# aukeschaap/ttcross

Measured on AMD Instinct MI355X. Metric: fiber evals/s (neval / wall time of dtt_dmrgg), Ising C_64 n=51 r=32 piv=2 (d=63), higher is better.
Workload: dtype f64; 1 GPU; Ising C_64 n=51 r=32 piv=2 (d=63); driver=test_crs_ising c 64 51 32 2, bond_groups=8, transport=none (single process), arith=exact, sweeps=16

## Files before the change

### ttcross_amd/csrc/ttx_cluster.h

```cpp
#pragma once
#include "ttx_fused.h"
#include "ttx_mvn.h"

#define CB 256
#ifndef TTX_CL_UNR
#define TTX_CL_UNR 16
#endif

__device__ __forceinline__ double f_ising_c4p(int m, int A, const double *an, const double *aw, double s1n, double s1w,
                                              double s2n, double s2w, const double *bn, const double *bw,
                                              double pv, double pvk, double pw, double pwk)
{
    const int nb = m - A - 2;
    double v = pv, w = pw, vk = pvk, wk = pwk;
    auto vstep = [&](double xv) { vk = vk * xv; v = v + vk; };
    auto wstep = [&](double xv) { wk = wk * xv; w = w + wk; };
    vstep(s2n); vstep(s1n);
    chain8v<true>(an, A, vstep);
    wstep(s1n); wstep(s2n);
    chain8v<false>(bn, nb, wstep);
    double b = 1.0 / (v * w);
    double f = 2 * b;
    auto fstep = [&](double xv) { f = f * xv; };
    chain8v<false>(aw, A, fstep);
    fstep(s1w); fstep(s2w);
    chain8v<false>(bw, nb, fstep);
    return f;
}

template <class STEP>
__device__ __forceinline__ void chain8w(const double *p, int nc, STEP step)
{
#pragma unroll 1
    for (int ch = 0; ch < nc; ch++) {
        double x[8];
        ld8d(p + 8 * ch, x);
#pragma unroll
        for (int k = 0; k < 8; k++) step(x[k]);
    }
}
__device__ __forceinline__ double f_ising_c4w(int cA, int cB, const double *an, const double *aw, double s1n, double s1w,
                                              double s2n, double s2w, const double *bn, const double *bw,
                                              double pv, double pvk, double pw, double pwk)
{
    double v = pv, w = pw, vk = pvk, wk = pwk;
    auto vstep = [&](double xv) { vk = vk * xv; v = v + vk; };
    auto wstep = [&](double xv) { wk = wk * xv; w = w + wk; };
    vstep(s2n); vstep(s1n);
    chain8w(an, cA, vstep);
    wstep(s1n); wstep(s2n);
    chain8w(bn, cB, wstep);
    double b = 1.0 / (v * w);
    double f = 2 * b;
    auto fstep = [&](double xv) { f = f * xv; };
    chain8w(aw, cA, fstep);
    fstep(s1w); fstep(s2w);
    chain8w(bw, cB, fstep);
    return f;
}

__device__ __forceinline__ int wave_min_i(int v)
{
    v = min(v, __builtin_amdgcn_update_dpp(INT_MAX, v, 0xb1, 0xf, 0xf, false));
    v = min(v, __builtin_amdgcn_update_dpp(INT_MAX, v, 0x4e, 0xf, 0xf, false));
    v = min(v, __builtin_amdgcn_update_dpp(INT_MAX, v, 0x124, 0xf, 0xf, false));
    v = min(v, __builtin_amdgcn_update_dpp(INT_MAX, v, 0x128, 0xf, 0xf, false));
    v = min(v, __builtin_amdgcn_update_dpp(INT_MAX, v, 0x142, 0xa, 0xf, false));
    v = min(v, __builtin_amdgcn_update_dpp(INT_MAX, v, 0x143, 0xc, 0xf, false));
    return __builtin_amdgcn_readlane(v, 63);
}
__device__ __forceinline__ void wave_argmax2(double &a, double &v, int &idx)
{
    const double amx = wave_max(a);
    const int key = (a == amx && idx != INT_MAX) ? ((idx << 1) | (signbit(v) ? 1 : 0)) : INT_MAX;
    const int kmin = wave_min_i(key);
    a = amx;
    if (kmin == INT_MAX) { idx = INT_MAX; v = 0.0; }
    else { idx = kmin >> 1; v = (kmin & 1) ? -amx : amx; }
}

__device__ __forceinline__ double f_ising_cfast(double xj, double wj, double xk, double wk, double pv, double pvk, double pw, double pwk,
                                                double SL, double WL, double SR, double WR)
{
    const double v = pv + pvk * xk * (1.0 + xj * (1.0 + SL));
    const double w = pw + pwk * xj * (1.0 + xk * (1.0 + SR));
    return 2.0 / (v * w) * ((WL * wj) * (wk * WR));
}

typedef unsigned int u4 __attribute__((ext_vector_type(4)));
struct ClRec { u4 a, b; };
static_assert(sizeof(ClRec) == sizeof(ClPart), "record buffers are sized as ClPart: [2][G][TTX_CLREC] u4 arg-max records, then as many running-maximum records");
__device__ __forceinline__ void st16(void *p, u4 v) { asm volatile("global_store_dwordx4 %0, %1, off sc1" :: "v"(p), "v"(v) : "memory"); }
__device__ __forceinline__ u4 ld16(const void *p)
{
    u4 v;
    asm volatile("global_load_dwordx4 %0, %1, off sc1\n\ts_waitcnt vmcnt(0)" : "=v"(v) : "v"(p) : "memory");
    return v;
}

__device__ __forceinline__ int xcc_id() { return (int)__builtin_amdgcn_s_getreg(((4 - 1) << 11) | 20) & 15; }
__global__ void k_xcc_probe(int *out) { if (threadIdx.x == 0) out[blockIdx.x] = xcc_id(); }

__device__ __forceinline__ bool cluster_sync(unsigned *ctr, unsigned target, int *abortflag, int *s_ok)
{
    asm volatile("s_waitcnt vmcnt(0)" ::: "memory");
    __syncthreads();
    if (threadIdx.x == 0) {
        int ok = 1;
        unsigned spins = 0;
        __hip_atomic_fetch_add(ctr, 1u, __ATOMIC_RELEASE, __HIP_MEMORY_SCOPE_AGENT);
        while (__hip_atomic_load(ctr, __ATOMIC_RELAXED, __HIP_MEMORY_SCOPE_AGENT) < target) {
            __builtin_amdgcn_s_sleep(1);
            if (++spins > (1u << 22)) { ok = 0; __hip_atomic_store(abortflag, 1, __ATOMIC_RELAXED, __HIP_MEMORY_SCOPE_SYSTEM); break; }
            if ((spins & 1023u) == 0 && __hip_atomic_load(abortflag, __ATOMIC_RELAXED, __HIP_MEMORY_SCOPE_SYSTEM)) { ok = 0; break; }
        }
        __atomic_thread_fence(__ATOMIC_ACQUIRE);
        *s_ok = ok;
    }
    __syncthreads();
    return *s_ok != 0;
}

#ifdef TTX_STAMPS
#define CST_DECL const bool t_me = (threadIdx.x == 0 && g == 0 && cb == 0); long long t_prev = wall_clock64()
#define CST(k) do { if (t_me) { long long t_now = wall_clock64(); gs.stamp[0][k] += t_now - t_prev; t_prev = t_now; } } while (0)
#define CST_END() do { if (t_me) gs.nstamp[0]++; } while (0)
#define WST(k) do { if (P.dbg && g == 0 && epoch == 8 && pp == 4 && lane == 0 && h < 8) P.dbg[((size_t)(h * 64 + cb * 4 + wv)) * 8 + (k)] = (long long)__builtin_readcyclecounter(); } while (0)
#else
#define WST(k)
#define CST_DECL
#define CST(k)
#define CST_END()
#endif

template <bool CFAST, bool CPAD>
__global__ __launch_bounds__(CB) void k_sweep_cluster(DevProb P, int dir, int nsteps, int NB, int ldsinv, int epoch, int zkeep)
{
    extern __shared__ __align__(16) double dyn[];
    __shared__ int zc[128], zr[128], zcs[128], zrs[128], keepc[128], keepr[128];
    __shared__ int nzc, nzr, nsc, nsr, s_ok;
    __shared__ ttx_cdfseg segc[TTX_TABSEG], segr[TTX_TABSEG];
    __shared__ double sha[8], shv[8], shm[8]; __shared__ int shi[8];
    __shared__ double pLw[64], pLk[64], pRv[64], pRk[64];
    static_assert(!(CFAST && CPAD), "the closed form reads the rows in dimension order");
    constexpr int NFT = CFAST ? 64 : 1;
    __shared__ double fSL[NFT], fWL[NFT], fSR[NFT], fWR[NFT];
    __shared__ struct { int ii, jj, kk, qq, hcount, rc_k, rc_q, rr_i, rr_j; double pivot, amax, bytes_half; long long neval, n_resid; } s_rook;
    const int bid = blockIdx.x;
    const int g = (bid & 7) + 8 * (bid / (8 * NB)), cb = (bid >> 3) % NB;
    if (g >= P.G || P.ctl[0]) return;
    const int bpar = (epoch - 1) & 1;
    if (P.tail_side && epoch >= 2) {
        const TailRec &t0 = P.tailrec[(size_t)bpar * P.G];
        if (stop_rule(epoch - 1, P.maxrank, P.accuracy, t0.pivotmax, max_pos(t0.amax, P.gs[0].amax_bnd[bpar]), P.strk[epoch & 1]).ready) return;
    }
    if (P.cl_test_abort && P.cl_test_abort == epoch && g == 0 && cb == 0) {
        if (threadIdx.x == 0) { __hip_atomic_store(P.cl_abort, 1, __ATOMIC_RELAXED, __HIP_MEMORY_SCOPE_SYSTEM); P.ctl[0] = 1; }
        return;
    }
    const int tid = threadIdx.x, m = P.d, RM = P.RM, NM = P.NM;
    const int lane = tid & 63, wv = tid >> 6;
    GroupState &gs = P.gs[g];
    const int first = gs.first, last = gs.last, nbonds = last - first + 1;
    int *r = P.r + (size_t)g * (m + 2);
    const int VS = ((m + 7) & ~7) + 8;
    const int RS = 2 * VS + 2;
    const int n1m = P.n[1];
    const int SL = RM * ((NM + NB - 1) / NB + 1);
    unsigned *ctr = P.cl_ctr + g;
    unsigned nbar = (unsigned)(epoch - 1) * (unsigned)min(nsteps, nbonds);
    ClPart *part = P.cl_part;
    double *par = dyn;
    double *XL = par + ((P.npar + 1) & ~1);
    double *XR = XL + (size_t)RM * RS;
    double *acol = XR + (size_t)RM * RS;
    double *arow = acol + SL;
    double *resc = arow + SL;
    double *resr = resc + SL;
    double *xsc = resr + SL;
    double *xsr = xsc + ((RM + 1) & ~1);
    int *lot = (int *)(xsr + ((RM + 1) & ~1));
    double *GL = (double *)(lot + 4 * ((2 * RM + 2 * NM + 4 + 1) & ~1));
    double *GU = GL + (size_t)RM * RM;
    int *ZK = (int *)(ldsinv ? GU + (size_t)RM * RM : GL);
    int *ZN = ZK + (size_t)nsteps * 2 * RM;
    for (int x = tid; x < P.npar; x += CB) par[x] = P.par[x];
    if (cb == 0 && tid == 0) sweep_start(P, g);
    __syncthreads();
    if (zkeep) {
        int *TMP = (int *)XL;
        const int E = nbonds * 2 * RM;
        for (int x = tid; x < E; x += CB) {
            const int b = x / (2 * RM), side = (x / RM) & 1, u = x % RM, pb = first + b;
            if (u < r[pb]) { const int *vp = vip_ptr(P, g, pb, first) + 4 * u; TMP[x] = (vp[2 * side + 1] << 16) | vp[2 * side]; }
        }
        __syncthreads();
        for (int x = tid; x < E; x += CB) {
            const int b = x / (2 * RM), u = x % RM, nb_ = r[first + b];
            if (u < nb_) {
                const int *src = TMP + (x - u); const int a = src[u]; int ra = 0;
                for (int t = 0; t < nb_; t++) ra += (src[t] < a) || (src[t] == a && t < u);
                ZK[(x - u) + ra] = a;
            }
        }
        __syncthreads();
        for (int x = tid; x < E; x += CB) {
            const int b = x / (2 * RM), u = x % RM, nb_ = r[first + b];
            if (u < nb_) {
                const int *src = ZK + (x - u); int pc = 0;
                for (int t = 1; t <= u; t++) pc += (src[t] != src[t - 1]);
                const bool keep = (u == 0) || (src[u] != src[u - 1]);
                TMP[x] = keep ? pc : -1;
                if (u == nb_ - 1) ZN[x / RM] = pc + 1;
            }
        }
        __syncthreads();
        int mykey = 0, mypos = -1;
        for (int x0 = 0; x0 < E; x0 += CB) {
            const int x = x0 + tid;
            mypos = -1;
            if (x < E) { const int b = x / (2 * RM), u = x % RM; if (u < r[first + b]) { mypos = TMP[x]; mykey = ZK[x]; } }
            __syncthreads();
            if (mypos >= 0) ZK[(x - x % RM) + mypos] = mykey;
            __syncthreads();
        }
    }
    double amax = gs.amax, pivotmax = -1.0, pivotmin = -1.0;
    if (P.tail_side && epoch >= 2) amax = max_pos(amax, gs.amax_bnd[bpar]);
    const double pivotmax_prev = gs.pivotmax_prev;
    long long neval = gs.neval;
    unsigned long long rngpos = gs.rngpos;
    double bytes_half = gs.bytes_half; long long n_resid = gs.n_resid;
    int hcount = 0;
    const unsigned long long bil0 = ttx_minstd_pow(2ull * tid);
    unsigned long long sA0 = ttx_minstd_pow(2 * rngpos + 1);
    const int bl0 = (int)ttx_minstd_pow(2ull * lane);
    const unsigned long long c64 = ttx_minstd_pow(128);
    CST_DECL;

    for (int pp = 1; pp <= nsteps; pp++) {
        if (pp > nbonds) break;
        const int p = (dir == 1) ? first + pp - 1 : last + 1 - pp;
        const int r0 = r[p - 1], r1 = r[p], r2 = r[p + 1], n1 = P.n[p], n2 = P.n[p + 1];
        const int nlot = r0 + n1 + n2 + r2;
        auto slice = [&](int c, int n) { return (int)((unsigned)c * (unsigned)n / (unsigned)NB); };
        const int jlo = slice(cb, n1), jhi = slice(cb + 1, n1);
        const int klo = slice(cb, n2), khi = slice(cb + 1, n2);
        const int nj = jhi - jlo, nk = khi - klo;
        double *Cp = core_ptr(P, P.col, g, p, first), *Wq = core_ptr(P, P.row, g, p + 1, first);
        double *Ap = core_ptr(P, P.arg, g, p, first), *Aq = core_ptr(P, P.arg, g, p + 1, first);
        const short *Lt = L_ptr(P, g, p - 1, first), *Rt = R_ptr(P, g, p + 1, first);
        const int cA = (p - 1 + 7) >> 3, cB = (m - p - 1 + 7) >> 3;
        const int sside = (tid >> 6) & 1, sseg = tid & 63;
        double sg_a0 = 0.0, sg_al = 0.0, sg_de = 0.0; int sg_k0 = 0, sg_cn = 0, myns = 0;
        auto seg_issue = [&](int Kc_, int Kr_) {
            if (tid >= 128) {
                const int K = sside ? Kr_ : Kc_; const ttx_cdfseg *sp = P.cdf_tab + (size_t)K * TTX_TABSEG + sseg;
                myns = P.cdf_ns[K]; sg_a0 = sp->a0; sg_al = sp->alast; sg_de = sp->delta; sg_k0 = sp->k0; sg_cn = sp->cnt;
            }
        };
        {
            const int AL = min(VS, (p - 1 + 7) & ~7), AR = min(VS, (m - p - 1 + 7) & ~7);
            if (AL > 0) {
                int c = tid / AL, o = tid - c * AL;
                const int dc = CB / AL, dO = CB - dc * AL;
                while (c < r0) {
                    if constexpr (CPAD) {
                        if (o < p - 1) {
                            const int ix = (int)Lt[(size_t)o * RM + c];
                            XL[(size_t)c * RS + (p - 2 - o)] = par[ix - 1]; XL[(size_t)c * RS + VS + o] = par[n1m + ix - 1];
                        } else { XL[(size_t)c * RS + o] = 0.0; XL[(size_t)c * RS + VS + o] = 1.0; }
                    } else {
                        const int ix = (o < p - 1) ? (int)Lt[(size_t)o * RM + c] : 1;
                        XL[(size_t)c * RS + o] = par[ix - 1]; XL[(size_t)c * RS + VS + o] = par[n1m + ix - 1];
                    }
                    c += dc; o += dO; if (o >= AL) { o -= AL; c++; }
                }
            }
            if (AR > 0) {
                int c = tid / AR, o = tid - c * AR;
                const int dc = CB / AR, dO = CB - dc * AR;
                while (c < r2) {
                    if (CPAD && o >= m - p - 1) { XR[(size_t)c * RS + o] = 0.0; XR[(size_t)c * RS + VS + o] = 1.0; }
                    else {
                        const int ix = (o < m - p - 1) ? (int)Rt[(size_t)o * RM + c] : 1;
                        XR[(size_t)c * RS + o] = par[ix - 1]; XR[(size_t)c * RS + VS + o] = par[n1m + ix - 1];
                    }
                    c += dc; o += dO; if (o >= AR) { o -= AR; c++; }
                }
            }
        }
        if (ldsinv) {
            if (p > first) { const double *gL = inv_ptr(P, g, p - 1, first); for (int x = tid; x < r0 * r0; x += CB) GL[x] = gL[x]; }
            if (p < last)  { const double *gU = inv_ptr(P, g, p + 1, first); for (int x = tid; x < r2 * r2; x += CB) GU[x] = gU[x]; }
        }
        CST(0);
        if (zkeep) seg_issue(r0 * n1 - ZN[2 * (p - first)], n2 * r2 - ZN[2 * (p - first) + 1]);
        if (tid == 0) s_ok = 1;
        unsigned long long stepmul;
        if (nlot < 512) {
            stepmul = (unsigned long long)(unsigned)__shfl(bl0, nlot & 63);
            for (int a = 0; a < (nlot >> 6); a++) stepmul = ttx_mulmod31(stepmul, c64);
        } else stepmul = ttx_minstd_pow(2ull * nlot);
        const unsigned long long sA1 = ttx_mulmod31(sA0, stepmul);
        if (zkeep) {
            const int b = p - first;
            const int *kc = ZK + (size_t)b * 2 * RM, *kr = kc + RM;
            if (tid == 0) { nzc = ZN[2 * b]; nzr = ZN[2 * b + 1]; }
            if (tid < ZN[2 * b]) zc[tid] = ((kc[tid] & 0xffff) - 1) + r0 * ((kc[tid] >> 16) - 1) + 1;
            if (tid < ZN[2 * b + 1]) zr[tid] = ((kr[tid] & 0xffff) - 1) + n2 * ((kr[tid] >> 16) - 1) + 1;
            __syncthreads();
        } else bond_zero_lists(vip_ptr(P, g, p, first), r1, r0, n2, tid, zc, zr, zcs, zrs, keepc, keepr, &nzc, &nzr);
        CST(1);
        const int Kc = r0 * n1 - nzc, Kr = n2 * r2 - nzr;
        if (!zkeep) seg_issue(Kc, Kr);
        if (tid >= 128) {
            ttx_cdfseg *dst = sside ? segr : segc;
            if (sseg < myns) { dst[sseg].a0 = sg_a0; dst[sseg].alast = sg_al; dst[sseg].delta = sg_de; dst[sseg].k0 = sg_k0; dst[sseg].cnt = sg_cn; }
            if (sseg == 0) { if (sside) nsr = myns; else nsc = myns; }
        }
        if (tid < r0) {
            double w = 1.0, wk = 1.0;
            auto wstep = [&](double xv) { wk = wk * xv; w = w + wk; };
            if constexpr (CPAD) chain8v<true>(XL + (size_t)tid * RS, p - 1, wstep);
            else chain8v<false>(XL + (size_t)tid * RS, p - 1, wstep);
            pLw[tid] = w; pLk[tid] = wk;
            if constexpr (CFAST) {
                double sk = 1.0, ss = 0.0, ww = 1.0;
                auto sstep = [&](double xv) { sk = sk * xv; ss = ss + sk; };
                auto pstep = [&](double xv) { ww = ww * xv; };
                chain8v<true>(XL + (size_t)tid * RS, p - 1, sstep);
                chain8v<false>(XL + (size_t)tid * RS + VS, p - 1, pstep);
                fSL[tid] = ss; fWL[tid] = ww;
            }
        } else if (tid >= 64 && tid < 64 + r2) {
            const int c = tid - 64;
            double v = 1.0, vk = 1.0;
            auto vstep = [&](double xv) { vk = vk * xv; v = v + vk; };
            chain8v<true>(XR + (size_t)c * RS, m - p - 1, vstep);
            pRv[c] = v; pRk[c] = vk;
            if constexpr (CFAST) {
                double sk = 1.0, ss = 0.0, ww = 1.0;
                auto sstep = [&](double xv) { sk = sk * xv; ss = ss + sk; };
                auto pstep = [&](double xv) { ww = ww * xv; };
                chain8v<false>(XR + (size_t)c * RS, m - p - 1, sstep);
                chain8v<false>(XR + (size_t)c * RS + VS, m - p - 1, pstep);
                fSR[c] = ss; fWR[c] = ww;
            }
        }
        __syncthreads();
        CST(2);
        double ma = 0.0, ba = -1.0, bv = 0.0; int bi = INT_MAX;
        const int nscu = __builtin_amdgcn_readfirstlane(nsc), nsru = __builtin_amdgcn_readfirstlane(nsr);
        const int nzcu = __builtin_amdgcn_readfirstlane(nzc), nzru = __builtin_amdgcn_readfirstlane(nzr);
        for (int il = tid; il < nlot; il += CB) {
            const unsigned long long bil = (il == tid) ? bil0 : ttx_minstd_pow(2ull * il);
            const double d1 = ttx_flang_from_word(ttx_mulmod31(sA0, bil)), d2 = ttx_flang_from_word(ttx_mulmod31(sA1, bil));
            const ttx_pair xy = ttx_lottery_index2<TTX_TABSEG, 64>(segc, nscu, Kc, r0 * n1, zc, nzcu, d1, segr, nsru, Kr, n2 * r2, zr, nzru, d2);
            const int x = xy.x, y = xy.y;
            CST(3);
            const int i = (x - 1) % r0 + 1, j = (x - 1) / r0 + 1, k = (y - 1) % n2 + 1, q = (y - 1) / n2 + 1;
            lot[4 * il] = i; lot[4 * il + 1] = j; lot[4 * il + 2] = k; lot[4 * il + 3] = q;
            const double *rl = XL + (size_t)(i - 1) * RS, *rq = XR + (size_t)(q - 1) * RS;
            double f;
            if constexpr (CFAST) f = f_ising_cfast(par[j - 1], par[n1m + j - 1], par[k - 1], par[n1m + k - 1], pRv[q - 1], pRk[q - 1], pLw[i - 1], pLk[i - 1], fSL[i - 1], fWL[i - 1], fSR[q - 1], fWR[q - 1]);
            else if constexpr (CPAD) f = f_ising_c4w(cA, cB, rl, rl + VS, par[j - 1], par[n1m + j - 1], par[k - 1], par[n1m + k - 1], rq, rq + VS, pRv[q - 1], pRk[q - 1], pLw[i - 1], pLk[i - 1]);
            else f = f_ising_c4p(m, p - 1, rl, rl + VS, par[j - 1], par[n1m + j - 1], par[k - 1], par[n1m + k - 1], rq, rq + VS, pRv[q - 1], pRk[q - 1], pLw[i - 1], pLk[i - 1]);
            ma = fmax(ma, fabs(f));
            CST(4);
            const double *c = Cp + (i - 1) + (size_t)RM * (j - 1), *w = Wq + (k - 1) + (size_t)NM * (q - 1);
            double t = 0.0;
#pragma unroll 8
            for (int s = 0; s < r1; s++) t = t + c[P.SS * s] * w[P.SW * s];
            const double b = f - t, aa = fabs(b);
            if (aa > ba || (aa == ba && il < bi)) { ba = aa; bv = b; bi = il; }
        }
        ma = wave_max(ma);
        wave_argmax(ba, bv, bi);
        if (lane == 0) { shm[wv] = ma; sha[wv] = ba; shv[wv] = bv; shi[wv] = bi; }
        __syncthreads();
        ma = shm[0]; ba = sha[0]; bv = shv[0]; bi = shi[0];
        for (int x = 1; x < CB / 64; x++) {
            ma = fmax(ma, shm[x]);
            if (sha[x] > ba || (sha[x] == ba && shi[x] < bi)) { ba = sha[x]; bv = shv[x]; bi = shi[x]; }
        }
        amax = fmax(amax, ma);
        neval += nlot; rngpos += 2ull * nlot;
        sA0 = ttx_mulmod31(sA1, stepmul);
        if (bi == INT_MAX) bi = 0;
        int ii = lot[4 * bi], jj = lot[4 * bi + 1], kk = lot[4 * bi + 2], qq = lot[4 * bi + 3];
        double pivot = bv;
        CST(5);
        int havecol = 0, haverow = 0, crs = 0, done = 0;
        int rc_k = -1, rc_q = -1, rr_i = -1, rr_j = -1;
        const int H = (P.piv == 0) ? 2 : 2 * P.piv;
        const int r1u = __builtin_amdgcn_readfirstlane(r1);
        double mxrun = 0.0;
        auto wact = [&](int c) {
            const int njc = slice(c + 1, n1) - slice(c, n1), nkc = slice(c + 1, n2) - slice(c, n2);
            const int e = max(r0 * njc, nkc * r2);
            return min(CB / 64, max(1, (e + 63) >> 6));
        };
        const bool rook_active = wv < wact(cb);
        const bool slot_on = (lane < NB * (CB / 64)) && ((lane & (CB / 64 - 1)) < wact(lane / (CB / 64)));
        if (rook_active) {
        for (int h = 0; h < H && !done; h++) {
            const bool iscol = (P.piv == 0) ? (h == 0) : (((h + (dir == 2 ? 1 : 0)) & 1) == 0);
            const int nf = iscol ? r0 * n1 : n2 * r2;
            const int nsl = iscol ? r0 * nj : nk * r2;
            double *fib = iscol ? acol : arow;
            double xsv = 0.0;
            if (lane < r1) xsv = iscol ? Wq[(kk - 1) + (size_t)NM * (qq - 1) + P.SW * lane] : Cp[(ii - 1) + (size_t)RM * (jj - 1) + P.SS * lane];
            crs++;
            if (iscol) havecol = 1; else haverow = 1;
            const int dn = (P.piv == 0) ? (h == 1) : (havecol && haverow && (crs >= 2 * P.piv));
            const bool resid = (P.piv != 0) && !dn;
            if (iscol) { rc_k = resid ? kk : -1; rc_q = qq; } else { rr_i = resid ? ii : -1; rr_j = jj; }
            CST(6);
            WST(0);
            double mx = 0.0, ab = -1.0, bb = 0.0; int ix = INT_MAX;
            for (int u = tid; u < nsl; u += CB) {
                double a;
                if (iscol) {
                    const int i = u % r0, j = jlo + u / r0, t = i + r0 * j;
                    const double *rl = XL + (size_t)i * RS, *rq = XR + (size_t)(qq - 1) * RS;
                    const double *c = Cp + i + (size_t)RM * j;
                    if constexpr (CFAST) a = f_ising_cfast(par[j], par[n1m + j], par[kk - 1], par[n1m + kk - 1], pRv[qq - 1], pRk[qq - 1], pLw[i], pLk[i], fSL[i], fWL[i], fSR[qq - 1], fWR[qq - 1]);
                    else if constexpr (CPAD) a = f_ising_c4w(cA, cB, rl, rl + VS, par[j], par[n1m + j], par[kk - 1], par[n1m + kk - 1], rq, rq + VS, pRv[qq - 1], pRk[qq - 1], pLw[i], pLk[i]);
                    else a = f_ising_c4p(m, p - 1, rl, rl + VS, par[j], par[n1m + j], par[kk - 1], par[n1m + kk - 1], rq, rq + VS, pRv[qq - 1], pRk[qq - 1], pLw[i], pLk[i]);
                    fib[u] = a;
                    if (resid) {
                        double b = a;
#pragma unroll TTX_CL_UNR
                        for (int s = 0; s < r1u; s++) b = b + (-mvn_lane(xsv, s)) * c[P.SS * s];
                        resc[u] = b;
                        const double aa = fabs(b);
                        if (aa > ab || (aa == ab && t < ix)) { ab = aa; bb = b; ix = t; }
                    }
                } else {
                    const int k = klo + u % nk, q = u / nk, t = k + n2 * q;
                    const double *rl = XL + (size_t)(ii - 1) * RS, *rq = XR + (size_t)q * RS;
                    const double *w = Wq + k + (size_t)NM * q;
                    if constexpr (CFAST) a = f_ising_cfast(par[jj - 1], par[n1m + jj - 1], par[k], par[n1m + k], pRv[q], pRk[q], pLw[ii - 1], pLk[ii - 1], fSL[ii - 1], fWL[ii - 1], fSR[q], fWR[q]);
                    else if constexpr (CPAD) a = f_ising_c4w(cA, cB, rl, rl + VS, par[jj - 1], par[n1m + jj - 1], par[k], par[n1m + k], rq, rq + VS, pRv[q], pRk[q], pLw[ii - 1], pLk[ii - 1]);
                    else a = f_ising_c4p(m, p - 1, rl, rl + VS, par[jj - 1], par[n1m + jj - 1], par[k], par[n1m + k], rq, rq + VS, pRv[q], pRk[q], pLw[ii - 1], pLk[ii - 1]);
                    fib[u] = a;
                    if (resid) {
                        double tt = 0.0;
#pragma unroll TTX_CL_UNR
                        for (int s = 0; s < r1u; s++) tt = tt + w[P.SW * s] * mvn_lane(xsv, s);
                        const double b = a + (-1.0) * tt;
                        resr[u] = b;
                        const double aa = fabs(b);
                        if (aa > ab || (aa == ab && t < ix)) { ab = aa; bb = b; ix = t; }
                    }
                }
                mx = fmax(mx, fabs(a));
            }
            CST(7);
            WST(1);
            mx = wave_max(mx);
            wave_argmax2(ab, bb, ix);
            WST(2);
            u4 *bufA = (u4 *)part + ((size_t)(hcount & 1) * P.G + g) * TTX_CLREC;
            u4 *bufB = bufA + (size_t)2 * P.G * TTX_CLREC;
            const unsigned gen = ((unsigned)epoch << 20) | (unsigned)(hcount + 1);
            mxrun = fmax(mxrun, mx);
            if (lane == 0) {
                const unsigned long long ua = (unsigned long long)__double_as_longlong(ab), um = (unsigned long long)__double_as_longlong(mxrun);
                u4 ra, rb;
                rb.x = (unsigned)um; rb.y = (unsigned)(um >> 32); rb.z = gen; rb.w = 0;
                st16(&bufB[cb * (CB / 64) + wv], rb);
                ra.x = (unsigned)ua; ra.y = (unsigned)(ua >> 32); ra.z = (unsigned)ix; ra.w = gen | (signbit(bb) ? 0x80000000u : 0u);
                st16(&bufA[cb * (CB / 64) + wv], ra);
            }
            CST(8);
            WST(3);
            int ok = 1;
            ab = -1.0; bb = 0.0; ix = INT_MAX;
            if (slot_on) {
                unsigned spins = 0;
                for (;;) {
                    const u4 ra = ld16(&bufA[lane]);
                    if ((ra.w & 0x7fffffffu) == gen) {
                        ab = __longlong_as_double((long long)(((unsigned long long)ra.y << 32) | ra.x));
                        ix = (int)ra.z;
                        bb = (ra.w & 0x80000000u) ? -ab : ab;
                        break;
                    }
                    if (++spins > 64u) __builtin_amdgcn_s_sleep(1);
                    if (spins > (1u << 22)) { ok = 0; break; }
                    if ((spins & 1023u) == 0 && __hip_atomic_load(P.cl_abort, __ATOMIC_RELAXED, __HIP_MEMORY_SCOPE_SYSTEM)) { ok = 0; break; }
                }
            }
            WST(4);
            ok = __all(ok);
            wave_argmax2(ab, bb, ix);
            WST(5);
            if (!ok) {
                if (lane == 0) { __hip_atomic_store(P.cl_abort, 1, __ATOMIC_RELAXED, __HIP_MEMORY_SCOPE_SYSTEM); P.ctl[0] = 1; *(volatile int *)&s_ok = 0; }
                return;
            }
            CST(9);
            hcount++;
            neval += nf;
            bytes_half += resid ? 8.0 * ((double)nf * r1 + r1 + 2.0 * nf) : 8.0 * nf;
            n_resid += resid ? 1 : 0;
            done = dn;
            if (resid) {
                if (ix == INT_MAX) ix = 0;
                if (iscol) { const int i = ix % r0 + 1, j = ix / r0 + 1; done = havecol && haverow && (i == ii && j == jj); ii = i; jj = j; }
                else       { const int k = ix % n2 + 1, q = ix / n2 + 1; done = havecol && haverow && (k == kk && q == qq); kk = k; qq = q; }
                pivot = bb;
            }
        }
        if (P.piv != 0) {
            u4 *bufB = (u4 *)part + ((size_t)((hcount - 1) & 1) * P.G + g) * TTX_CLREC + (size_t)2 * P.G * TTX_CLREC;
            const unsigned gen = ((unsigned)epoch << 20) | (unsigned)hcount;
            double mx = 0.0; int ok = 1;
            if (slot_on) {
                unsigned spins = 0;
                for (;;) {
                    const u4 rb = ld16(&bufB[lane]);
                    if (rb.z == gen) { mx = __longlong_as_double((long long)(((unsigned long long)rb.y << 32) | rb.x)); break; }
                    if (++spins > 64u) __builtin_amdgcn_s_sleep(1);
                    if (spins > (1u << 22)) { ok = 0; break; }
                    if ((spins & 1023u) == 0 && __hip_atomic_load(P.cl_abort, __ATOMIC_RELAXED, __HIP_MEMORY_SCOPE_SYSTEM)) { ok = 0; break; }
                }
            }
            ok = __all(ok);
            if (!ok) {
                if (lane == 0) { __hip_atomic_store(P.cl_abort, 1, __ATOMIC_RELAXED, __HIP_MEMORY_SCOPE_SYSTEM); P.ctl[0] = 1; *(volatile int *)&s_ok = 0; }
                return;
            }
            amax = fmax(amax, wave_max(mx));
        }
        if (tid == 0) {
            s_rook.ii = ii; s_rook.jj = jj; s_rook.kk = kk; s_rook.qq = qq; s_rook.hcount = hcount; s_rook.rc_k = rc_k; s_rook.rc_q = rc_q;
            s_rook.rr_i = rr_i; s_rook.rr_j = rr_j; s_rook.pivot = pivot; s_rook.amax = amax; s_rook.bytes_half = bytes_half; s_rook.neval = neval; s_rook.n_resid = n_resid;
        }
        }
        __syncthreads();
        if (!*(volatile int *)&s_ok) return;
        if (!rook_active) {
            ii = s_rook.ii; jj = s_rook.jj; kk = s_rook.kk; qq = s_rook.qq; hcount = s_rook.hcount; rc_k = s_rook.rc_k; rc_q = s_rook.rc_q;
            rr_i = s_rook.rr_i; rr_j = s_rook.rr_j; pivot = s_rook.pivot; amax = s_rook.amax; bytes_half = s_rook.bytes_half; neval = s_rook.neval; n_resid = s_rook.n_resid;
        }
        CST(10);
        int *tape = P.tape + ((size_t)g * (m + 2) + p) * 4;
        const bool upd = accept_pivot(pivot, amax, pivotmax_prev, P.small_element, P.small_pivot);
        if (!upd) {
            if (cb == 0 && tid == 0) { tape[0] = tape[1] = tape[2] = tape[3] = -1; P.upd[(size_t)g * (m + 2) + p] = 0; }
        } else {
            const int i0 = ii - 1, j0 = jj - 1, k0 = kk - 1, q0 = qq - 1;
            double *gI = inv_ptr(P, g, p, first);
            for (int s = tid; s < r1; s += CB) { xsc[s] = Wq[k0 + (size_t)NM * q0 + P.SW * s]; xsr[s] = Cp[i0 + (size_t)RM * j0 + P.SS * s]; }
            __syncthreads();
            if (cb == 0)
                for (int s = tid; s < r1; s += CB) { gI[r1 * r1 + s] = xsr[s]; gI[r1 * r1 + r1 + s] = xsc[s]; }
            const bool reuseA = (rc_k == kk && rc_q == qq), reuseB = (rr_i == ii && rr_j == jj);
            for (int u = tid; u < r0 * nj; u += CB) {
                const int i = u % r0, j = jlo + u / r0; const size_t o = i + (size_t)RM * j;
                const double a = acol[u];
                Ap[o + P.SS * r1] = a;
                double y;
                if (reuseA) y = resc[u];
                else {
                    y = a;
#pragma unroll 16
                    for (int s = 0; s < r1; s++) y = y + (-xsc[s]) * Cp[o + P.SS * s];
                }
                Cp[o + P.SS * r1] = (1.0 / pivot) * y;
            }
            for (int u = tid; u < nk * r2; u += CB) {
                const int k = klo + u % nk, q = u / nk;
                const double a = arow[u];
                Aq[r1 + (size_t)RM * k + P.SS * q] = a;
                const size_t o = k + (size_t)NM * q;
                if (reuseB) Wq[o + P.SW * r1] = resr[u];
                else {
                    double tt = 0.0;
#pragma unroll 16
                    for (int s = 0; s < r1; s++) tt = tt + Wq[o + P.SW * s] * xsr[s];
                    Wq[o + P.SW * r1] = a + (-1.0) * tt;
                }
            }
            CST(11);
            if (p > first) {
                const double *gL = ldsinv ? GL : inv_ptr(P, g, p - 1, first);
                double *Wp = core_ptr(P, P.row, g, p, first);
                const int pk = (r0 <= 32) ? 2 : 1, lw = 64 / pk, l = lane & (lw - 1), sub = lane / lw;
                for (int base = wv * pk; base < nj; base += (CB / 64) * pk) {
                    const int jl = base + sub, j = jlo + jl;
                    const bool on = (jl < nj) && (l < r0);
                    const double xf = wave_solve_L(gL, r0, on ? acol[l + r0 * jl] : 0.0, l, lw);
                    if (on) Wp[j + (size_t)NM * r1 + P.SW * l] = xf;
                }
            }
            CST(12);
            if (p < last) {
                const double *gU = ldsinv ? GU : inv_ptr(P, g, p + 1, first);
                double *Cq = core_ptr(P, P.col, g, p + 1, first);
                const int pk = (r2 <= 32) ? 2 : 1, lw = 64 / pk, l = lane & (lw - 1), sub = lane / lw;
                const double rdg = wave_solve_rdg(gU, r2, l);
                for (int base = wv * pk; base < nk; base += (CB / 64) * pk) {
                    const int kl = base + sub, k = klo + kl;
                    const bool on = (kl < nk) && (l < r2);
                    const double y = wave_solve_U(gU, r2, on ? arow[kl + nk * l] : 0.0, rdg, l, lw);
                    if (on) Cq[r1 + (size_t)RM * k + P.SS * l] = y;
                }
            }
            CST(13);
            if (cb == 0) {
                append_tables(P, g, p, first, r1, ii, jj, kk, qq, tid, CB);
                if (tid == 0) append_scalars(P, g, p, first, r1, ii, jj, kk, qq, pivot);
            }
            if (zkeep && wv < 2) {
                const int b = p - first;
                int *kl = ZK + (size_t)b * 2 * RM + (size_t)wv * RM;
                const int nl = ZN[2 * b + wv];
                const int key = wv == 0 ? ((jj << 16) | ii) : ((qq << 16) | kk);
                const int v = (lane < nl) ? kl[lane] : INT_MAX;
                const bool dup = __ballot(v == key) != 0ull;
                const int pos = __popcll(__ballot(v < key));
                if (!dup) {
                    if (lane < nl && v > key) kl[lane + 1] = v;
                    if (lane == 0) { kl[pos] = key; ZN[2 * b + wv] = nl + 1; }
                }
            }
            pivot_range(pivotmax, pivotmin, fabs(pivot));
        }
        CST(14);
        if (!cluster_sync(ctr, (++nbar) * (unsigned)NB, P.cl_abort, &s_ok)) { if (tid == 0) P.ctl[0] = 1; return; }
        CST(15);
        CST_END();
    }
    if (cb == 0) {
        if (tid == 0) {
            gs.amax = amax; gs.pivotmax = pivotmax; gs.pivotmin = pivotmin; gs.neval = neval; gs.rngpos = rngpos;
            gs.bytes_half = bytes_half; gs.n_resid = n_resid;
            if (P.tail_side) gs.amax_bnd[epoch & 1] = 0.0;
        }
        __syncthreads();
        exch_pack_group(P, g);
    }
}
```

Measured before the change: 214.9 million evals/s.

## Use integer-key wave max, precompute slice tables, skip argmax exchange on non-residual steps

Replaces the double wave_max with a two-pass integer DPP max over the high and low words of the bit pattern, which is valid for non-negative values. Slice bounds and active-wave counts are computed once per step by one wave into shared tables instead of per-thread division loops. In the rook loop, the argmax reductions and the cross-block argmax record exchange are skipped unless the step is residual (or piv==0), cutting atomic-polled traffic and spin waits. This relies on the inputs to the key max being non-negative and adds shared memory.

Measured after the change: 218.6 million evals/s, median of 6. 1.7% higher.

```diff
diff --git a/ttcross_amd/csrc/ttx_cluster.h b/ttcross_amd/csrc/ttx_cluster.h
--- a/ttcross_amd/csrc/ttx_cluster.h
+++ b/ttcross_amd/csrc/ttx_cluster.h
@@ -1,6 +1,7 @@
 #pragma once
 #include "ttx_fused.h"
 #include "ttx_mvn.h"
+#include "ttx_cluster_rules.h"
 
 #define CB 256
 #ifndef TTX_CL_UNR
@@ -69,9 +70,36 @@
     v = min(v, __builtin_amdgcn_update_dpp(INT_MAX, v, 0x143, 0xc, 0xf, false));
     return __builtin_amdgcn_readlane(v, 63);
 }
+__device__ __forceinline__ int wave_max_i(int v)
+{
+    v = max(v, __builtin_amdgcn_update_dpp(INT_MIN, v, 0xb1, 0xf, 0xf, false));
+    v = max(v, __builtin_amdgcn_update_dpp(INT_MIN, v, 0x4e, 0xf, 0xf, false));
+    v = max(v, __builtin_amdgcn_update_dpp(INT_MIN, v, 0x124, 0xf, 0xf, false));
+    v = max(v, __builtin_amdgcn_update_dpp(INT_MIN, v, 0x128, 0xf, 0xf, false));
+    v = max(v, __builtin_amdgcn_update_dpp(INT_MIN, v, 0x142, 0xa, 0xf, false));
+    v = max(v, __builtin_amdgcn_update_dpp(INT_MIN, v, 0x143, 0xc, 0xf, false));
+    return __builtin_amdgcn_readlane(v, 63);
+}
+__device__ __forceinline__ unsigned wave_max_u(unsigned v)
+{
+    v = max(v, (unsigned)__builtin_amdgcn_update_dpp(0, (int)v, 0xb1, 0xf, 0xf, false));
+    v = max(v, (unsigned)__builtin_amdgcn_update_dpp(0, (int)v, 0x4e, 0xf, 0xf, false));
+    v = max(v, (unsigned)__builtin_amdgcn_update_dpp(0, (int)v, 0x124, 0xf, 0xf, false));
+    v = max(v, (unsigned)__builtin_amdgcn_update_dpp(0, (int)v, 0x128, 0xf, 0xf, false));
+    v = max(v, (unsigned)__builtin_amdgcn_update_dpp(0, (int)v, 0x142, 0xa, 0xf, false));
+    v = max(v, (unsigned)__builtin_amdgcn_update_dpp(0, (int)v, 0x143, 0xc, 0xf, false));
+    return (unsigned)__builtin_amdgcn_readlane((int)v, 63);
+}
+__device__ __forceinline__ double wave_max_key(double x)
+{
+    const ClKey k = cl_key(x);
+    const int hmax = wave_max_i(k.hi);
+    const unsigned lmax = wave_max_u(cl_key_lo_at(k, hmax));
+    return cl_unkey(ClKey{hmax, lmax});
+}
 __device__ __forceinline__ void wave_argmax2(double &a, double &v, int &idx)
 {
-    const double amx = wave_max(a);
+    const double amx = wave_max_key(a);
     const int key = (a == amx && idx != INT_MAX) ? ((idx << 1) | (signbit(v) ? 1 : 0)) : INT_MAX;
     const int kmin = wave_min_i(key);
     a = amx;
@@ -139,6 +167,7 @@
     extern __shared__ __align__(16) double dyn[];
     __shared__ int zc[128], zr[128], zcs[128], zrs[128], keepc[128], keepr[128];
     __shared__ int nzc, nzr, nsc, nsr, s_ok;
+    __shared__ int slt[2][TTX_CLMAX + 1], wtab[TTX_CLMAX];
     __shared__ ttx_cdfseg segc[TTX_TABSEG], segr[TTX_TABSEG];
     __shared__ double sha[8], shv[8], shm[8]; __shared__ int shi[8];
     __shared__ double pLw[64], pLk[64], pRv[64], pRk[64];
@@ -243,10 +272,6 @@
         const int p = (dir == 1) ? first + pp - 1 : last + 1 - pp;
         const int r0 = r[p - 1], r1 = r[p], r2 = r[p + 1], n1 = P.n[p], n2 = P.n[p + 1];
         const int nlot = r0 + n1 + n2 + r2;
-        auto slice = [&](int c, int n) { return (int)((unsigned)c * (unsigned)n / (unsigned)NB); };
-        const int jlo = slice(cb, n1), jhi = slice(cb + 1, n1);
-        const int klo = slice(cb, n2), khi = slice(cb + 1, n2);
-        const int nj = jhi - jlo, nk = khi - klo;
         double *Cp = core_ptr(P, P.col, g, p, first), *Wq = core_ptr(P, P.row, g, p + 1, first);
         double *Ap = core_ptr(P, P.arg, g, p, first), *Aq = core_ptr(P, P.arg, g, p + 1, first);
         const short *Lt = L_ptr(P, g, p - 1, first), *Rt = R_ptr(P, g, p + 1, first);
@@ -296,6 +321,14 @@
         }
         CST(0);
         if (zkeep) seg_issue(r0 * n1 - ZN[2 * (p - first)], n2 * r2 - ZN[2 * (p - first) + 1]);
+        static_assert(2 * (TTX_CLMAX + 1) <= 64 && TTX_CLMAX + TTX_CLMAX + 2 < 64, "the two slice rows and the shuffles of the fill fit one wave");
+        if (wv == CB / 64 - 1) {
+            const int side = lane > TTX_CLMAX ? 1 : 0, c = lane - side * (TTX_CLMAX + 1);
+            const int s = cl_slice(min(c, NB), side ? n2 : n1, NB);
+            const int s1 = __shfl(s, lane + 1), t0 = __shfl(s, lane + TTX_CLMAX + 1), t1 = __shfl(s, lane + TTX_CLMAX + 2);
+            if (lane < 2 * (TTX_CLMAX + 1)) slt[side][c] = s;
+            if (lane < TTX_CLMAX) wtab[lane] = cl_wact(s1 - s, t1 - t0, r0, r2, CB / 64);
+        }
         if (tid == 0) s_ok = 1;
         unsigned long long stepmul;
         if (nlot < 512) {
@@ -350,6 +383,9 @@
         }
         __syncthreads();
         CST(2);
+        const int jlo = __builtin_amdgcn_readfirstlane(slt[0][cb]), jhi = __builtin_amdgcn_readfirstlane(slt[0][cb + 1]);
+        const int klo = __builtin_amdgcn_readfirstlane(slt[1][cb]), khi = __builtin_amdgcn_readfirstlane(slt[1][cb + 1]);
+        const int nj = jhi - jlo, nk = khi - klo;
         double ma = 0.0, ba = -1.0, bv = 0.0; int bi = INT_MAX;
         const int nscu = __builtin_amdgcn_readfirstlane(nsc), nsru = __builtin_amdgcn_readfirstlane(nsr);
         const int nzcu = __builtin_amdgcn_readfirstlane(nzc), nzru = __builtin_amdgcn_readfirstlane(nzr);
@@ -375,8 +411,8 @@
             const double b = f - t, aa = fabs(b);
             if (aa > ba || (aa == ba && il < bi)) { ba = aa; bv = b; bi = il; }
         }
-        ma = wave_max(ma);
-        wave_argmax(ba, bv, bi);
+        ma = wave_max_key(ma);
+        wave_argmax2(ba, bv, bi);
         if (lane == 0) { shm[wv] = ma; sha[wv] = ba; shv[wv] = bv; shi[wv] = bi; }
         __syncthreads();
         ma = shm[0]; ba = sha[0]; bv = shv[0]; bi = shi[0];
@@ -396,13 +432,8 @@
         const int H = (P.piv == 0) ? 2 : 2 * P.piv;
         const int r1u = __builtin_amdgcn_readfirstlane(r1);
         double mxrun = 0.0;
-        auto wact = [&](int c) {
-            const int njc = slice(c + 1, n1) - slice(c, n1), nkc = slice(c + 1, n2) - slice(c, n2);
-            const int e = max(r0 * njc, nkc * r2);
-            return min(CB / 64, max(1, (e + 63) >> 6));
-        };
-        const bool rook_active = wv < wact(cb);
-        const bool slot_on = (lane < NB * (CB / 64)) && ((lane & (CB / 64 - 1)) < wact(lane / (CB / 64)));
+        const bool rook_active = wv < wtab[cb];
+        const bool slot_on = (lane < NB * (CB / 64)) && ((lane & (CB / 64 - 1)) < wtab[lane / (CB / 64)]);
         if (rook_active) {
         for (int h = 0; h < H && !done; h++) {
             const bool iscol = (P.piv == 0) ? (h == 0) : (((h + (dir == 2 ? 1 : 0)) & 1) == 0);
@@ -459,9 +490,10 @@
             }
             CST(7);
             WST(1);
-            mx = wave_max(mx);
-            wave_argmax2(ab, bb, ix);
+            mx = wave_max_key(mx);
+            if (resid) wave_argmax2(ab, bb, ix);
             WST(2);
+            const bool xchg = resid || P.piv == 0;
             u4 *bufA = (u4 *)part + ((size_t)(hcount & 1) * P.G + g) * TTX_CLREC;
             u4 *bufB = bufA + (size_t)2 * P.G * TTX_CLREC;
             const unsigned gen = ((unsigned)epoch << 20) | (unsigned)(hcount + 1);
@@ -471,14 +503,16 @@
                 u4 ra, rb;
                 rb.x = (unsigned)um; rb.y = (unsigned)(um >> 32); rb.z = gen; rb.w = 0;
                 st16(&bufB[cb * (CB / 64) + wv], rb);
-                ra.x = (unsigned)ua; ra.y = (unsigned)(ua >> 32); ra.z = (unsigned)ix; ra.w = gen | (signbit(bb) ? 0x80000000u : 0u);
-                st16(&bufA[cb * (CB / 64) + wv], ra);
+                if (xchg) {
+                    ra.x = (unsigned)ua; ra.y = (unsigned)(ua >> 32); ra.z = (unsigned)ix; ra.w = gen | (signbit(bb) ? 0x80000000u : 0u);
+                    st16(&bufA[cb * (CB / 64) + wv], ra);
+                }
             }
             CST(8);
             WST(3);
             int ok = 1;
             ab = -1.0; bb = 0.0; ix = INT_MAX;
-            if (slot_on) {
+            if (xchg && slot_on) {
                 unsigned spins = 0;
                 for (;;) {
                     const u4 ra = ld16(&bufA[lane]);
@@ -495,7 +529,7 @@
             }
             WST(4);
             ok = __all(ok);
-            wave_argmax2(ab, bb, ix);
+            if (resid) wave_argmax2(ab, bb, ix);
             WST(5);
             if (!ok) {
                 if (lane == 0) { __hip_atomic_store(P.cl_abort, 1, __ATOMIC_RELAXED, __HIP_MEMORY_SCOPE_SYSTEM); P.ctl[0] = 1; *(volatile int *)&s_ok = 0; }
@@ -533,7 +567,7 @@
                 if (lane == 0) { __hip_atomic_store(P.cl_abort, 1, __ATOMIC_RELAXED, __HIP_MEMORY_SCOPE_SYSTEM); P.ctl[0] = 1; *(volatile int *)&s_ok = 0; }
                 return;
             }
-            amax = fmax(amax, wave_max(mx));
+            amax = fmax(amax, wave_max_key(mx));
         }
         if (tid == 0) {
             s_rook.ii = ii; s_rook.jj = jj; s_rook.kk = kk; s_rook.qq = qq; s_rook.hcount = hcount; s_rook.rc_k = rc_k; s_rook.rc_q = rc_q;
diff --git a/ttcross_amd/csrc/ttx_cluster_rules.h b/ttcross_amd/csrc/ttx_cluster_rules.h
--- /dev/null
+++ b/ttcross_amd/csrc/ttx_cluster_rules.h
@@ -0,0 +1,15 @@
+#pragma once
+#include "ttx_cdf.h"
+
+TTX_HD int cl_slice(int c, int n, int NB) { return (int)((unsigned)c * (unsigned)n / (unsigned)NB); }
+
+TTX_HD int cl_wact(int nj, int nk, int r0, int r2, int nw)
+{
+    const int a = r0 * nj, b = nk * r2, e = a > b ? a : b, w = (e + 63) >> 6;
+    return w < 1 ? 1 : (w > nw ? nw : w);
+}
+
+struct ClKey { int hi; unsigned lo; };
+TTX_HD ClKey cl_key(double x) { const uint64_t b = ttx_dbits(x); return ClKey{(int)(uint32_t)(b >> 32), (unsigned)b}; }
+TTX_HD double cl_unkey(ClKey k) { return ttx_bitsd(((uint64_t)(uint32_t)k.hi << 32) | k.lo); }
+TTX_HD unsigned cl_key_lo_at(ClKey k, int hmax) { return k.hi == hmax ? k.lo : 0u; }
```
